# liamliaw/medical-image-segmentation-with-visual-prompts

Measured on AMD Instinct MI355X. Metric: 3D volumes/sec (96^3, bf16) training step, higher is better.
Workload: dtype bf16; 1 GPU; cfg1: swin_unetr downstream, 1-ch 96^3, batch 4/GPU, window (7, 7, 7), enc_prompt=False, dec_prompt=False, dropout 0.0, random-init weights; global_batch=4, parallelism=dp1, launch=eager (one C-ABI call per kernel)

## Files before the change

### medical-image-segmentation-with-visual-prompts_amd/csrc/common.hpp

```cpp
#pragma once
#include <hip/hip_runtime.h>
#include <stdint.h>
#include <type_traits>
#include "../../include/mivp.h"

typedef __bf16 bf16_t;
typedef __bf16 bf16x8 __attribute__((ext_vector_type(8)));
typedef __bf16 bf16x4 __attribute__((ext_vector_type(4)));
typedef float f32x4 __attribute__((ext_vector_type(4)));

#define MIVP_DEV __device__ __forceinline__

MIVP_DEV f32x4 mfma16(bf16x8 a, bf16x8 b, f32x4 c) {
    return __builtin_amdgcn_mfma_f32_16x16x32_bf16(a, b, c, 0, 0, 0);
}
MIVP_DEV bf16x8 zero8() { bf16x8 z; for (int i = 0; i < 8; ++i) z[i] = (bf16_t)0.0f; return z; }
MIVP_DEV bf16x4 zero4() { bf16x4 z; for (int i = 0; i < 4; ++i) z[i] = (bf16_t)0.0f; return z; }
MIVP_DEV f32x4 fzero4() { f32x4 z = {0.f, 0.f, 0.f, 0.f}; return z; }

MIVP_DEV bf16x8 ld8(const bf16_t* p) { return *reinterpret_cast<const bf16x8*>(p); }
MIVP_DEV bf16x4 ld4(const bf16_t* p) { return *reinterpret_cast<const bf16x4*>(p); }
MIVP_DEV void st8(bf16_t* p, bf16x8 v) { *reinterpret_cast<bf16x8*>(p) = v; }
MIVP_DEV void st4(bf16_t* p, bf16x4 v) { *reinterpret_cast<bf16x4*>(p) = v; }

// ... 19 lines not shown
    const float v = match ? s : zero;
    return excl ? -INFINITY : v;
}
MIVP_DEV float classify_logit(float s, int kcls, int rq, bool& live, float zero) {
    return classify_logit_c<-1, -2>(s, kcls, rq, live, zero);
}
constexpr float MIVP_LOG2E = 1.4426950408889634f;
constexpr float MIVP_PAD_KEY_BIAS = -30000.0f;
constexpr float MIVP_LN2 = 0.6931471805599453f;

MIVP_DEV uint32_t drop_hash(uint32_t pair_idx, uint32_t key) {
    uint32_t t = pair_idx + key;
    t ^= t >> 16;
    t = __umul24(t, 0xB5AD4Fu);
    t ^= t >> 13;
    return __umul24(t, 0x6C62B9u) + (t >> 8) + ((key << 13) | (key >> 19));
}
MIVP_DEV uint32_t drop_seed(uint32_t seed, const uint32_t* __restrict__ epoch) {
    uint32_t s = epoch ? seed + epoch[0] * 0x9E3779B1u : seed;
    s ^= s >> 16; s *= 0x85EBCA6Bu;
    s ^= s >> 13; s *= 0xC2B2AE35u;
    return s ^ (s >> 16);
}
MIVP_DEV bool drop_keep(uint32_t h, int odd, uint32_t thr) { return ((odd ? (h >> 16) : (h & 0xFFFFu)) >= thr); }
MIVP_DEV uint32_t attn_row(long bph, int q, int Nqp, int Nkp) {
    return ((uint32_t)bph * (uint32_t)Nqp + (uint32_t)q) * (uint32_t)(Nkp >> 1);
}
MIVP_DEV uint32_t attn_pair(uint32_t row, int k) { return row + (uint32_t)(k >> 1); }

typedef unsigned u32x2 __attribute__((ext_vector_type(2)));
typedef unsigned u32x4 __attribute__((ext_vector_type(4)));
MIVP_DEV int sel(bool c, int a, int b) { return c ? a : b; }
MIVP_DEV long sel(bool c, long a, long b) { return c ? a : b; }
MIVP_DEV float sel(bool c, float a, float b) { return c ? a : b; }
MIVP_DEV bf16x4 keep_if(bf16x4 v, bool ok) {
    u32x2 u = __builtin_bit_cast(u32x2, v);
    const unsigned m = 0u - (unsigned)ok;
    u[0] &= m; u[1] &= m;
    return __builtin_bit_cast(bf16x4, u);
}
MIVP_DEV bf16x8 keep_if(bf16x8 v, bool ok) {
    u32x4 u = __builtin_bit_cast(u32x4, v);
    const unsigned m = 0u - (unsigned)ok;
    u[0] &= m; u[1] &= m; u[2] &= m; u[3] &= m;
    return __builtin_bit_cast(bf16x8, u);
}
struct FastDiv {
    uint32_t m, d;
    MIVP_DEV explicit FastDiv(int div) : m(0xFFFFFFFFu / (uint32_t)div + 1u), d((uint32_t)div) {}
    MIVP_DEV int div(int n) const { return d == 1u ? n : (int)__umulhi((uint32_t)n, m); }
    MIVP_DEV int mod(int n) const { return n - div(n) * (int)d; }
};

template <int DK>
struct OperandRows {
    static constexpr int ROW = DK == 32 ? 64 : (DK + 8) * 2;
    static MIVP_DEV int off(int row, int elem) {
        if (DK == 32) return row * 64 + 16 * ((elem >> 3) ^ ((0 - (row >> 2)) & 3)) + 2 * (elem & 7);
        return row * ROW + 2 * elem;
    }
};

MIVP_DEV bf16x8 wfrag(const bf16_t* __restrict__ wf, int ks, int nt, int s, int lane) {
    return ld8(wf + ((long)(nt * ks + s) * 64 + lane) * 8);
}
template <int KSL>
struct WeightSlabs {
    static constexpr int PCS = (64 * KSL + 255) / 256;
    static constexpr int BYTES = 2 * KSL * 1024;
    bf16x8 reg[PCS];
    MIVP_DEV void fetch(const bf16_t* __restrict__ wf, int nt) {
#pragma unroll
        for (int u = 0; u < PCS; ++u) reg[u] = ld8(wf + (long)nt * KSL * 512 + 8 * min((int)threadIdx.x + 256 * u, 64 * KSL - 1));
    }
    MIVP_DEV void store(char* smem, int buf) const {
#pragma unroll
        for (int u = 0; u < PCS; ++u)
            *reinterpret_cast<bf16x8*>(smem + buf * KSL * 1024 + 16 * min((int)threadIdx.x + 256 * u, 64 * KSL - 1)) = reg[u];
    }
    static MIVP_DEV bf16x8 frag(const char* smem, int buf, int s, int lane) {
        return *reinterpret_cast<const bf16x8*>(smem + buf * KSL * 1024 + s * 1024 + 16 * lane);
    }
};

template <int KSL>
struct WeightSlabsRM {
    static constexpr int PCS = (64 * KSL + 255) / 256;
    static constexpr int BYTES = 2 * KSL * 1024;
    bf16x8 reg[PCS];
    MIVP_DEV void fetch(const bf16_t* __restrict__ w, int ld, int row0, int nrows, int ncols) {
#pragma unroll
        for (int u = 0; u < PCS; ++u) {
            const int p = threadIdx.x + 256 * u;
            const int sub = p >> 6, row = row0 + ((p & 63) >> 2), col = 32 * sub + 8 * (p & 3);
            reg[u] = (p < 64 * KSL && row < nrows && col < ncols) ? ld8(w + (long)row * ld + col) : zero8();
        }
    }
    MIVP_DEV void store(char* smem, int buf) const {
#pragma unroll
        for (int u = 0; u < PCS; ++u) {
            const int p = threadIdx.x + 256 * u;
            if (p < 64 * KSL)
                *reinterpret_cast<bf16x8*>(smem + buf * KSL * 1024 + (p >> 6) * 1024 + OperandRows<32>::off((p & 63) >> 2, 8 * (p & 3))) = reg[u];
        }
    }
    static MIVP_DEV bf16x8 frag8(const char* smem, int buf, int sub, int r, int elem) {
// ... 52 lines not shown
```

### medical-image-segmentation-with-visual-prompts_amd/csrc/swin_fwd.hip

```cpp
#include "common.hpp"
#include <cstdlib>

int mivp_tok_wide_supported(const MivpSwinDesc* d);
int mivp_tok_rows_supported(const MivpSwinDesc* d);
long mivp_tok_natural_offset(int C);
int mivp_tok_wide_qkv_fwd(const MivpSwinDesc* d, const void* x, const int32_t* tok_src, const float* ln_w, const float* ln_b,
                          const void* wqkv, void* q, void* k, void* v, hipStream_t st);
int mivp_tok_wide_proj_mlp_fwd(const MivpSwinDesc* d, const void* o, const void* x, const int32_t* tok_src, const int32_t* tok_dst,
                               const void* wproj, const float* bproj, const float* ln_w, const float* ln_b, const void* wmlp,
                               const float* bmlp, void* t1_out, void* y, hipStream_t st);

template <int KS, bool CH12>
__global__ __launch_bounds__(256, 4) void k_swin_qkv_fwd(MivpSwinDesc d, const bf16_t* __restrict__ x,
                                                      const int* __restrict__ tok_src,
                                                      const float* __restrict__ ln_w, const float* __restrict__ ln_b,
                                                      const bf16_t* __restrict__ wqkv,
                                                      bf16_t* __restrict__ q, bf16_t* __restrict__ k,
                                                      bf16_t* __restrict__ v) {
    const int lane = threadIdx.x & 63, wave = __builtin_amdgcn_readfirstlane(threadIdx.x >> 6);
    const int r = lane & 15, g = lane >> 4;
    const int C = d.C, hd = C / d.heads;
    const long T = (long)d.B * d.P * d.Nqp;
    const long tile0 = ((long)blockIdx.x * 4 + wave) * 2;

    bf16x8 xb[2][KS];
    long bp[2];
    int slot[2];
    bool live[2];
#pragma unroll
    for (int u = 0; u < 2; ++u) {
        const long t = (tile0 + u) * 16 + r;
        live[u] = t < T;
        const unsigned tt = live[u] ? (unsigned)t : 0u;
        const unsigned bpu = tt / (unsigned)d.Nqp;
        bp[u] = bpu;
        slot[u] = (int)(tt - bpu * (unsigned)d.Nqp);
        const int pw = (int)(bpu % (unsigned)d.P);
        const long b = bpu / (unsigned)d.P;
        const int src = live[u] ? tok_src[pw * d.Nqp + slot[u]] : -2;
        float xs[KS][8];
        float sum = 0.f;
#pragma unroll
        for (int s = 0; s < KS; ++s) {
            const int c = 32 * s + 8 * g;
            if (src >= 0 && c < C) {
                bf16x8 raw = ld8(x + ((b * d.vol_in + src) * (long)C + c));
#pragma unroll
                for (int i = 0; i < 8; ++i) { xs[s][i] = (float)raw[i]; sum += xs[s][i]; }
            } else {
#pragma unroll
                for (int i = 0; i < 8; ++i) xs[s][i] = 0.f;
            }
        }
        const float mean = col_sum(sum) / (float)C;
        float var = 0.f;
#pragma unroll
        for (int s = 0; s < KS; ++s) {
            if (32 * s + 8 * g < C) {
// ... 83 lines not shown
    using WR = OperandRows<32>;
    bf16x8 wreg[PCS];
    auto slab_fetch = [&](int nt) {
#pragma unroll
        for (int u = 0; u < PCS; ++u) {
            wreg[u] = ld8(wqkv + (long)nt * KS * 512 + 8 * min((int)threadIdx.x + 256 * u, 64 * KS - 1));
        }
    };
    auto slab_store = [&](int buf) {
#pragma unroll
        for (int u = 0; u < PCS; ++u) {
            *reinterpret_cast<bf16x8*>(wsm + buf * KS * 1024 + 16 * min((int)threadIdx.x + 256 * u, 64 * KS - 1)) = wreg[u];
        }
    };
    if (LDSW && nt_begin < nt_end) { slab_fetch(nt_begin); slab_store(0); __syncthreads(); }
    int o_sel = (16 * nt_begin + 4 * g) / C;
    int o_head = ((16 * nt_begin + 4 * g) - o_sel * C) / hd;
    int o_j0 = (16 * nt_begin + 4 * g) - o_sel * C - o_head * hd;
    for (int nt = nt_begin; nt < nt_end; ++nt) {
        f32x4 acc0 = fzero4(), acc1 = fzero4();
        const int nrow = 16 * nt + r;
        if (LDSW) {
            const int cur = (nt - nt_begin) & 1;
            if (nt + 1 < nt_end) slab_fetch(nt + 1);
            const char* slab = wsm + cur * KS * 1024;
#pragma unroll
            for (int s = 0; s < KS; ++s) {
                const bf16x8 a = *reinterpret_cast<const bf16x8*>(slab + s * 1024 + 16 * lane);
                acc0 = mfma16(a, xb[0][s], acc0);
                acc1 = mfma16(a, xb[1][s], acc1);
            }
            if (nt + 1 < nt_end) slab_store(cur ^ 1);
            __syncthreads();
        } else {
#pragma unroll
            for (int s = 0; s < KS; ++s) {
                const bf16x8 a = wfrag(wqkv, KS, nt, s, lane);
                acc0 = mfma16(a, xb[0][s], acc0);
                acc1 = mfma16(a, xb[1][s], acc1);
            }
        }
        const int n0 = 16 * nt + 4 * g;
        if (n0 < n_out) {
            while (o_j0 >= hd) { o_j0 -= hd; ++o_head; }
            while (o_head >= d.heads) { o_head -= d.heads; ++o_sel; }
            const int sel = o_sel, head = o_head, j0 = o_j0;
            o_j0 += 16;
            bf16_t* base = sel == 0 ? q : (sel == 1 ? k : v);
            const float sc = sel == 0 ? d.q_scale : (sel == 1 ? MIVP_LOG2E : 1.0f);
            if (live[0]) st4(base + ((bp[0] * d.heads + head) * d.Nqp + slot[0]) * (long)hd + j0, pack4(acc0 * sc));
            if (live[1]) st4(base + ((bp[1] * d.heads + head) * d.Nqp + slot[1]) * (long)hd + j0, pack4(acc1 * sc));
        }
    }
}

__global__ __launch_bounds__(256) void k_prompt_kv_fwd(MivpSwinDesc d, const float* __restrict__ prompt,
                                                       const float* __restrict__ ln_w, const float* __restrict__ ln_b,
                                                       const bf16_t* __restrict__ wqkv, bf16_t* __restrict__ kp,
                                                       bf16_t* __restrict__ vp, float* __restrict__ yln) {
    extern __shared__ __attribute__((aligned(16))) char smem[];
    float* y = reinterpret_cast<float*>(smem);
    float* red = y + d.C;
    const int t = blockIdx.x, C = d.C, hd = C / d.heads;
    const int tid = threadIdx.x;
    if (t >= d.Np) {
        for (int n = tid; n < 2 * C; n += 256) {
            const int sel = n / C, cc = n - sel * C, head = cc / hd, j = cc - head * hd;
            (sel == 0 ? kp : vp)[((long)head * d.Npp + t) * hd + j] = (bf16_t)0.0f;
        }
        return;
    }
    float part = 0.f;
    for (int c = tid; c < C; c += 256) part += prompt[(long)t * C + c];
    for (int o = 32; o > 0; o >>= 1) part += __shfl_xor(part, o);
    if ((tid & 63) == 0) red[tid >> 6] = part;
    __syncthreads();
    const float mean = (red[0] + red[1] + red[2] + red[3]) / (float)C;
    __syncthreads();
    part = 0.f;
    for (int c = tid; c < C; c += 256) { const float dv = prompt[(long)t * C + c] - mean; part += dv * dv; }
    for (int o = 32; o > 0; o >>= 1) part += __shfl_xor(part, o);
    if ((tid & 63) == 0) red[4 + (tid >> 6)] = part;
    __syncthreads();
    const float rstd = rsqrtf((red[4] + red[5] + red[6] + red[7]) / (float)C + d.ln_eps);
    for (int c = tid; c < C; c += 256) {
        const float yy = (prompt[(long)t * C + c] - mean) * rstd * ln_w[c] + ln_b[c];
        if (yln) yln[(long)t * C + c] = yy;
        y[c] = (float)(bf16_t)yy;
    }
    __syncthreads();
    for (int n = tid; n < 2 * C; n += 256) {
        const int sel = n / C, cc = n - sel * C;
        const bf16_t* wrow = wqkv + (long)((sel + 1) * C + cc) * C;
        float acc = 0.f;
        for (int c = 0; c < C; ++c) acc += y[c] * (float)wrow[c];
        const int head = cc / hd, j = cc - head * hd;
        (sel == 0 ? kp : vp)[((long)head * d.Npp + t) * hd + j] = (bf16_t)(sel == 0 ? acc * MIVP_LOG2E : acc);
    }
}

struct PromptKvJob {
    MivpSwinDesc d;
    const float* prompt; const float* ln_w; const float* ln_b; const bf16_t* wqkv; const float* ts;
    bf16_t* kp; bf16_t* vp; bf16_t* ka;
};
struct PromptKvJobs { PromptKvJob job[16]; };
// ... 658 lines not shown
            const int n0 = 16 * nt + 4 * g;
            const f32x4 w4 = *reinterpret_cast<const f32x4*>(ln_w + min(n0, C - 4));
            const f32x4 b4 = *reinterpret_cast<const f32x4*>(ln_b + min(n0, C - 4));
#pragma unroll
            for (int j = 0; j < 4; ++j) yy[j] = (bf16_t)((t1[nt][j] - mean) * rstd * w4[j] + b4[j]);
            yy = keep_if(yy, n0 < C);
        }
        y2[nt] = yy;
    }
    if (LDSW) { slab_fetch(wmlp, 0); slab_store(0); __syncthreads(); }
#pragma unroll
    for (int mt = 0; mt < CT; ++mt) {
        f32x4 acc = fzero4();
        const int nrow = 16 * mt + r;
        if (LDSW) {
            if (mt + 1 < CT) slab_fetch(wmlp, mt + 1);
            const char* slab = wsm + (mt & 1) * KS * 1024;
#pragma unroll
            for (int s = 0; s < KS; ++s) {
                acc = mfma16(*reinterpret_cast<const bf16x8*>(slab + s * 1024 + 16 * lane), cat44(y2[2 * s], y2[2 * s + 1]), acc);
            }
            if (mt + 1 < CT) slab_store((mt + 1) & 1);
            __syncthreads();
        } else {
#pragma unroll
            for (int s = 0; s < KS; ++s) {
                acc = mfma16(wfrag(wmlp, KS, mt, s, lane), cat44(y2[2 * s], y2[2 * s + 1]), acc);
            }
        }
        const int n0 = 16 * mt + 4 * g;
        const f32x4 bm4 = *reinterpret_cast<const f32x4*>(bmlp + min(n0, C - 4));
        if (n0 < C && dst >= 0) {
#pragma unroll
            for (int j = 0; j < 4; ++j) acc[j] += t1[mt][j] + bm4[j];
            st4(y + ((b * d.vol_out + dst) * (long)C + n0), pack4(acc));
        }
    }
}

static int swin_common_checks(const MivpSwinDesc* d) {
    MIVP_REQUIRE(d != nullptr);
    MIVP_REQUIRE(d->B > 0 && d->C > 0 && d->heads > 0 && d->P > 0);
    MIVP_REQUIRE(d->C % 8 == 0 && d->C % d->heads == 0 && (d->C / d->heads) % 4 == 0);
    MIVP_REQUIRE(d->Nqp % 16 == 0 && d->Nqp >= d->Nq && d->Nqp - d->Nq < 16);
    MIVP_REQUIRE((long)d->B * d->P * d->Nqp < (1L << 31));
    MIVP_REQUIRE(d->Npp % 16 == 0 && d->Npp >= d->Np);
    MIVP_REQUIRE(d->Nkp % 32 == 0 && d->Nkp >= d->Nqp + d->Npp);
    MIVP_REQUIRE(d->augp % 4 == 0 && d->augp >= d->aug);
    MIVP_REQUIRE(d->aug == d->win[0] + d->win[1] + d->win[2] - 1);
    MIVP_REQUIRE(d->Nq == d->win[0] * d->win[1] * d->win[2]);
    return MIVP_OK;
}

extern "C" int mivp_swin_qkv_fwd(const MivpSwinDesc* d, const void* x, const int32_t* tok_src, const float* ln_w,
                                 const float* ln_b, const void* wqkv, void* q, void* k, void* v,
                                 mivp_stream_t stream) {
    int rc = swin_common_checks(d);
    if (rc) return rc;
    MIVP_REQUIRE(x && tok_src && ln_w && ln_b && wqkv && q && k && v);
    if (mivp_tok_wide_supported(d)) return mivp_tok_wide_qkv_fwd(d, x, tok_src, ln_w, ln_b, wqkv, q, k, v, (hipStream_t)stream);
    const long T = (long)d->B * d->P * d->Nqp;
    const unsigned gx = (unsigned)((T + 127) / 128);
    const int KS = (d->C + 31) / 32;
    const int n_tiles = (3 * d->C + 15) / 16;
    int nsplit = (int)((4096 + 4L * gx - 1) / (4L * gx));
    if (nsplit > n_tiles / 3) nsplit = n_tiles / 3;
    if (nsplit < 1) nsplit = 1;
    const dim3 grid(gx, (unsigned)nsplit);
    hipStream_t st = (hipStream_t)stream;
#define LAUNCH_QKV2(K, CH) hipLaunchKernelGGL((k_swin_qkv_fwd<K, CH>), grid, dim3(256), 0, st, *d, (const bf16_t*)x, tok_src, \
                                              ln_w, ln_b, (const bf16_t*)wqkv, (bf16_t*)q, (bf16_t*)k, (bf16_t*)v)
#define LAUNCH_QKV(K) LAUNCH_QKV2(K, false)
    const bool ch12 = d->C == 48 && d->heads == 4 && nsplit == 1 && d->Nqp % 32 == 0;
    switch (KS) {
        case 1: LAUNCH_QKV(1); break;
        case 2: if (ch12) LAUNCH_QKV2(2, true); else LAUNCH_QKV(2); break;
        case 3: LAUNCH_QKV(3); break;
        case 4: LAUNCH_QKV(4); break;
        case 6: LAUNCH_QKV(6); break;
        default: mivp_set_error("swin_qkv_fwd: C/32 not in {1,2,3,4,6}"); return MIVP_EUNSUPPORTED;
    }
#undef LAUNCH_QKV
    return mivp_check_launch("swin_qkv_fwd");
}

extern "C" int mivp_prompt_kv_fwd(const MivpSwinDesc* d, const float* prompt, const float* ln_w, const float* ln_b,
                                  const void* wqkv, void* kp, void* vp, float* yln, mivp_stream_t stream) {
    int rc = swin_common_checks(d);
    if (rc) return rc;
    MIVP_REQUIRE(d->Np > 0 && prompt && ln_w && ln_b && wqkv && kp && vp);
    hipLaunchKernelGGL(k_prompt_kv_fwd, dim3(d->Npp), dim3(256), (d->C + 8) * sizeof(float), (hipStream_t)stream, *d,
                       prompt, ln_w, ln_b, (const bf16_t*)wqkv, (bf16_t*)kp, (bf16_t*)vp, yln);
    return mivp_check_launch("prompt_kv_fwd");
}

extern "C" int mivp_prompt_kv_fwd_multi(int32_t n, const MivpSwinDesc* d, const float* const* prompt, const float* const* ln_w,
                                        const float* const* ln_b, const void* const* wqkv, const float* const* ts,
                                        void* const* kp, void* const* vp, void* const* ka, mivp_stream_t stream) {
    MIVP_REQUIRE(n > 0 && n <= 16 && d && prompt && ln_w && ln_b && wqkv && ts && kp && vp && ka);
    PromptKvJobs jobs;
    int rows = 0;
    size_t lds = 0;
    for (int i = 0; i < n; ++i) {
        int rc = swin_common_checks(&d[i]);
        if (rc) return rc;
        MIVP_REQUIRE(d[i].Np > 0 && prompt[i] && ln_w[i] && ln_b[i] && wqkv[i] && ts[i] && kp[i] && vp[i] && ka[i]);
        jobs.job[i] = PromptKvJob{d[i], prompt[i], ln_w[i], ln_b[i], (const bf16_t*)wqkv[i], ts[i], (bf16_t*)kp[i], (bf16_t*)vp[i],
                                  (bf16_t*)ka[i]};
        rows = d[i].Npp > rows ? d[i].Npp : rows;
        const size_t need = (d[i].C + 8) * sizeof(float);
        lds = need > lds ? need : lds;
    }
    hipLaunchKernelGGL(k_prompt_kv_fwd_multi, dim3(rows, n), dim3(256), lds, (hipStream_t)stream, jobs);
    return mivp_check_launch("prompt_kv_fwd_multi");
}

extern "C" int mivp_relbias_aug(const MivpSwinDesc* d, const float* t_h, const float* t_w, const float* t_d,
                                const float* ts, void* qa, void* ka, mivp_stream_t stream) {
    int rc = swin_common_checks(d);
    if (rc) return rc;
    MIVP_REQUIRE(t_h && t_w && t_d && qa && ka);
    MIVP_REQUIRE(d->Np == 0 || ts != nullptr);
    hipLaunchKernelGGL(k_relbias_aug, dim3(d->heads + 1, 8), dim3(256), 0, (hipStream_t)stream, *d, t_h, t_w, t_d, ts,
                       (bf16_t*)qa, (bf16_t*)ka);
    return mivp_check_launch("relbias_aug");
}
// ... 107 lines not shown
```

### medical-image-segmentation-with-visual-prompts_amd/csrc/swin_tok_wide.hip

```cpp
#include "common.hpp"
#include <cstdlib>

namespace {

template <int CT>
struct WideGeom {
    static constexpr int C = 16 * CT;
    static constexpr int KP = (C + 31) / 32 * 32;
    static constexpr int KS = KP / 32;
    static constexpr int NCG = (CT % 4 == 0) ? 4 : (CT % 2 == 0 ? 2 : 1);
    static constexpr int NTG = 4 / NCG;
    static constexpr int NCT = CT / NCG;
    static constexpr int ROWS = 32 * NTG;
    static constexpr int TPR = 256 / ROWS;
    static constexpr int XPT = C / 8 / TPR;
    static_assert(CT % NCG == 0 && (C / 8) % TPR == 0, "even splits");
};

template <int K>
struct RowImg {
    static constexpr int ROWB = 2 * K + 16;
    static MIVP_DEV bf16x8 frag(const char* img, int row, int k0) { return *reinterpret_cast<const bf16x8*>(img + row * ROWB + 2 * k0); }
    static MIVP_DEV bf16x4 get4(const char* img, int row, int k0) { return *reinterpret_cast<const bf16x4*>(img + row * ROWB + 2 * k0); }
    static MIVP_DEV void put4(char* img, int row, int k0, bf16x4 v) { *reinterpret_cast<bf16x4*>(img + row * ROWB + 2 * k0) = v; }
    static MIVP_DEV void put8(char* img, int row, int k0, bf16x8 v) { *reinterpret_cast<bf16x8*>(img + row * ROWB + 2 * k0) = v; }
};

struct RowTok { long tt, bp, b; int slot, pw; bool live; };
MIVP_DEV RowTok row_token(const MivpSwinDesc& d, long t) {
    RowTok ti;
    const long T = (long)d.B * d.P * d.Nqp;
    ti.live = t < T;
    const unsigned tu = ti.live ? (unsigned)t : 0u;
    const unsigned bpu = tu / (unsigned)d.Nqp;
    ti.tt = tu;
    ti.bp = bpu;
    ti.slot = (int)(tu - bpu * (unsigned)d.Nqp);
    ti.pw = (int)(bpu % (unsigned)d.P);
    ti.b = bpu / (unsigned)d.P;
    return ti;
}
template <int TPR>
MIVP_DEV float row_sum(float v) {
#pragma unroll
    for (int o = 1; o < TPR; o <<= 1) v += __shfl_xor(v, o);
    return v;
}
MIVP_DEV void to_f32(bf16x8 v, float (&out)[8]) {
#pragma unroll
    for (int e = 0; e < 8; ++e) out[e] = (float)v[e];
}

template <int CT>
struct FlatRows {
    using G = WideGeom<CT>;
    static constexpr int PPR = G::C / 8, N = G::XPT;
    static_assert(G::ROWS * PPR == 256 * N, "pieces split evenly over the threads");
    int prow[N], col[N];
    RowTok tk[N];
    MIVP_DEV FlatRows(const MivpSwinDesc& d, long row0, int tid) {
#pragma unroll
        for (int i = 0; i < N; ++i) {
            const int P = tid + 256 * i;
            prow[i] = P / PPR;
            col[i] = 8 * (P - prow[i] * PPR);
            tk[i] = row_token(d, row0 + prow[i]);
        }
    }
};
template <int CT> constexpr bool flat_rows() { return CT == 3; }

template <int C, int NTG>
struct HeadMajor {
    long gbase[NTG];
    bool glive[NTG];
    int hd, hd4, heads;
    long head_stride;
    FastDiv by_chunk, by_hd4, by_heads;
    static constexpr int PER_GRAN = 24 * C;
    static constexpr int PPT = PER_GRAN * NTG / 256;
    MIVP_DEV HeadMajor(const MivpSwinDesc& d, long row0)
        : hd(C / d.heads), hd4(C / d.heads / 4), heads(d.heads), head_stride((long)d.Nqp * (C / d.heads)),
          by_chunk(8 * (C / d.heads)), by_hd4(C / d.heads / 4), by_heads(d.heads) {
        const long T = (long)d.B * d.P * d.Nqp;
#pragma unroll
        for (int gi = 0; gi < NTG; ++gi) {
            const long t0 = row0 + 32 * gi;
            glive[gi] = t0 < T;
            const unsigned tu = glive[gi] ? (unsigned)t0 : 0u;
            const unsigned bp = tu / (unsigned)d.Nqp, slot0 = tu - bp * (unsigned)d.Nqp;
            gbase[gi] = ((long)bp * heads * d.Nqp + slot0) * hd;
        }
    }
    template <class F>
    MIVP_DEV void each(int tid, F&& visit) const {
#pragma unroll
        for (int i = 0; i < PPT; ++i) {
            const int P = tid + 256 * i;
            const int gran = P / PER_GRAN, pg = P - gran * PER_GRAN;
// ... 348 lines not shown
            for (int e = 0; e < 8; ++e) sum += ts[i][e];
        }
        const float mean = row_sum<TPR>(sum) / (float)C;
        float var = 0.f;
#pragma unroll
        for (int i = 0; i < XPT; ++i)
#pragma unroll
            for (int e = 0; e < 8; ++e) { const float dvv = ts[i][e] - mean; var += dvv * dvv; }
        const float rstd = rsqrtf(row_sum<TPR>(var) / (float)C + d.ln_eps);
#pragma unroll
        for (int i = 0; i < XPT; ++i) {
            const int c = 8 * (sub + TPR * i);
            const f32x4 w0 = *reinterpret_cast<const f32x4*>(ln_w + c), w1 = *reinterpret_cast<const f32x4*>(ln_w + c + 4);
            const f32x4 b0 = *reinterpret_cast<const f32x4*>(ln_b + c), b1 = *reinterpret_cast<const f32x4*>(ln_b + c + 4);
            bf16x8 yy;
#pragma unroll
            for (int e = 0; e < 4; ++e) {
                yy[e] = (bf16_t)((ts[i][e] - mean) * rstd * w0[e] + b0[e]);
                yy[4 + e] = (bf16_t)((ts[i][4 + e] - mean) * rstd * w1[e] + b1[e]);
            }
            RI::put8(Aimg, row, c, yy);
        }
    }
    __syncthreads();
    {
#pragma unroll
        for (int j = 0; j < NCT; ++j) {
            const int nt = cg + NCG * j, n0 = 16 * nt + 4 * g;
            const f32x4 bm4 = *reinterpret_cast<const f32x4*>(bmlp + n0);
            f32x4 a0 = fzero4(), a1 = fzero4();
#pragma unroll
            for (int s = 0; s < KS; ++s) {
                bf16x8 a;
                if constexpr (PREW) a = wa[j][s]; else a = wfrag(wmlp, KS, nt, s, lane);
                a0 = mfma16(a, RI::frag(Aimg, R0, 32 * s + 8 * g), a0);
                a1 = mfma16(a, RI::frag(Aimg, R1, 32 * s + 8 * g), a1);
            }
            RI::put4(Ximg, R0, n0, pack4(a0 + t1[j][0] + bm4));
            RI::put4(Ximg, R1, n0, pack4(a1 + t1[j][1] + bm4));
        }
    }
    __syncthreads();
    if (FLAT) {
#pragma unroll
        for (int i = 0; i < XPT; ++i) {
            const int P = tid + 256 * i, prow = P / (C / 8), col = 8 * (P - prow * (C / 8));
            if (fdst[i] >= 0) st8(y + ((long)fb[i] * d.vol_out + fdst[i]) * (long)C + col, RI::frag(Ximg, prow, col));
        }
    } else if (dst >= 0) {
        const long yoff = (ti.b * d.vol_out + dst) * (long)C;
#pragma unroll
        for (int i = 0; i < XPT; ++i) st8(y + yoff + 8 * (sub + TPR * i), RI::frag(Ximg, row, 8 * (sub + TPR * i)));
    }
}

template <int CT>
__global__ __launch_bounds__(256, 3) void k_proj_mlp_bwd_wide(MivpSwinDesc d, const bf16_t* __restrict__ dy, const int* __restrict__ tok_dst,
                                                              const bf16_t* __restrict__ t1, const float* __restrict__ ln_w,
                                                              const bf16_t* __restrict__ wmlp_t, const bf16_t* __restrict__ wproj_t,
                                                              bf16_t* __restrict__ d_o, bf16_t* __restrict__ d_t1) {
    using G = WideGeom<CT>;
    constexpr int C = G::C, KS = G::KS, ROWS = G::ROWS, TPR = G::TPR, NCG = G::NCG, NCT = G::NCT, XPT = G::XPT;
    using RI = RowImg<G::KP>;
    extern __shared__ __attribute__((aligned(16))) char smem[];
    char* Dimg = smem;
    char* Timg = Dimg + ROWS * RI::ROWB;
    float* stat = reinterpret_cast<float*>(Timg + ROWS * RI::ROWB);
    float* red = stat + 2 * ROWS;
    const int tid = threadIdx.x, lane = tid & 63, wave = __builtin_amdgcn_readfirstlane(tid >> 6);
    const int r = lane & 15, g = lane >> 4;
    const long row0 = (long)blockIdx.x * ROWS;
    const int row = tid / TPR, sub = tid % TPR;
    const RowTok ti = row_token(d, row0 + row);
    const uint32_t proj_key = drop_seed(d.proj_seed, d.seed_epoch);
    const bool drop = d.proj_drop_thr != 0;
    {
        const int dst = sel(ti.live, tok_dst[ti.pw * d.Nqp + ti.slot], -1);
        const long yoff = (ti.b * d.vol_out + max(dst, 0)) * (long)C;
        bf16x8 dr[XPT], tr[XPT];
#pragma unroll
        for (int i = 0; i < XPT; ++i) {
            dr[i] = ld8(dy + yoff + 8 * (sub + TPR * i));
            tr[i] = ld8(t1 + ti.tt * (long)C + 8 * (sub + TPR * i));
        }
        float ts[XPT][8], sum = 0.f;
#pragma unroll
        for (int i = 0; i < XPT; ++i) {
            const bf16x8 tv = keep_if(tr[i], ti.live);
            RI::put8(Dimg, row, 8 * (sub + TPR * i), keep_if(dr[i], dst >= 0));
            RI::put8(Timg, row, 8 * (sub + TPR * i), tv);
            to_f32(tv, ts[i]);
#pragma unroll
            for (int e = 0; e < 8; ++e) sum += ts[i][e];
        }
        const float mean = row_sum<TPR>(sum) / (float)C;
        float var = 0.f;
#pragma unroll
        for (int i = 0; i < XPT; ++i)
#pragma unroll
            for (int e = 0; e < 8; ++e) { const float dvv = ts[i][e] - mean; var += dvv * dvv; }
        const float rstd = rsqrtf(row_sum<TPR>(var) / (float)C + d.ln_eps);
        if (sub == 0) {
            stat[2 * row] = mean;
            stat[2 * row + 1] = rstd;
            for (int c = C; c < G::KP; c += 8) { RI::put8(Dimg, row, c, zero8()); RI::put8(Timg, row, c, zero8()); }
        }
// ... 326 lines not shown
    PackJobs jobs;
    jobs.n = 0;
    jobs.C = C;
    jobs.w[0] = wq; jobs.w[1] = wk; jobs.w[2] = wv; jobs.w[3] = wproj; jobs.w[4] = wmlp;
    const int ct = (C + 15) / 16, ks = (C + 31) / 32, ks3 = (3 * 16 * ct + 31) / 32, ct3 = (3 * C + 15) / 16;
    auto add = [&](void* out, int src, int transposed, int kind, int rows, int cols, int k_steps) {
        if (!out) return;
        PackJob& j = jobs.job[jobs.n++];
        j.out = (bf16_t*)out; j.src = src; j.transposed = transposed; j.kind = kind; j.rows = rows; j.cols = cols; j.k_steps = k_steps;
        j.elems = kind == 0 ? (long)rows * cols : (long)((rows + 15) / 16) * k_steps * 512;
    };
    const long img = (long)ct * ks * 512;
    add(wqkv_rm, 0, 0, 0, 3 * C, C, 0);
    add(wqkv_f, 0, 0, 1, 3 * C, C, ks);
    add(wproj_f, 1, 0, 1, C, C, ks);
    add(wmlp_f, 2, 0, 2, C, C, ks);
    if (with_natural && wmlp_f) add((bf16_t*)wmlp_f + img, 2, 0, 1, C, C, ks);
    add(wqkv_t, 0, 1, 1, C, 3 * C, ks3);
    add(wmlp_t, 2, 1, 1, C, C, ks);
    add(wproj_t, 1, 1, 2, C, C, ks);
    if (with_natural && wproj_t) add((bf16_t*)wproj_t + img, 1, 1, 1, C, C, ks);
    (void)ct3;
    long total = 0;
    for (int j = 0; j < jobs.n; ++j) total += jobs.job[j].elems;
    if (total == 0) return MIVP_OK;
    const unsigned grid = (unsigned)((total + 255) / 256 < 4096 ? (total + 255) / 256 : 4096);
    hipLaunchKernelGGL(k_pack_block_weights, dim3(grid), dim3(256), 0, (hipStream_t)stream, jobs);
    return mivp_check_launch("pack_block_weights");
}

extern "C" int mivp_pack_weight_frags(const void* w, int32_t rows, int32_t cols, int32_t k_steps, int32_t paired, void* out,
                                      mivp_stream_t stream) {
    MIVP_REQUIRE(w && out && rows > 0 && cols > 0 && k_steps >= (cols + 31) / 32);
    const long total = (long)((rows + 15) / 16) * k_steps * 512;
    const unsigned grid = (unsigned)((total + 255) / 256 < 2048 ? (total + 255) / 256 : 2048);
    hipLaunchKernelGGL(k_pack_weight_frags, dim3(grid), dim3(256), 0, (hipStream_t)stream, (const bf16_t*)w, rows, cols, k_steps,
                       paired, (bf16_t*)out, total);
    return mivp_check_launch("pack_weight_frags");
}

int mivp_tok_wide_supported(const MivpSwinDesc* d) {
    const int hd = d->C / d->heads;
    if (!(d->C == 48 || d->C == 96 || d->C == 192 || d->C == 384)) return 0;
    static const bool off = getenv("MIVP_NO_WIDE_TOKEN_KERNELS") != nullptr;
    if (off) return 0;
    if (d->C == 48 && !getenv("MIVP_C48_QKV_ROW_KERNELS")) return 0;
    return (hd % 4 == 0 && d->Nqp % 32 == 0 && 8 * hd < 65536 && 72 * d->C < 65536) ? 1 : 0;
}
int mivp_tok_rows_supported(const MivpSwinDesc* d) {
    if (mivp_tok_wide_supported(d)) return 1;
    static const bool off = getenv("MIVP_NO_WIDE_TOKEN_KERNELS") != nullptr;
    return (!off && d->C == 48) ? 1 : 0;
}
long mivp_tok_natural_offset(int C) { return (long)(C / 16) * ((C + 31) / 32) * 512; }

#define ROWS_SWITCH(LAUNCH)                                                                  \
    switch (d->C) {                                                                          \
        case 48: LAUNCH(3); break;                                                           \
        case 96: LAUNCH(6); break;                                                           \
        case 192: LAUNCH(12); break;                                                         \
        case 384: LAUNCH(24); break;                                                         \
        default: mivp_set_error("tok_rows: C not in {48, 96, 192, 384}"); return MIVP_EUNSUPPORTED; \
    }
#define WIDE_SWITCH(LAUNCH)                                                                  \
    switch (d->C) {                                                                          \
        case 96: LAUNCH(6); break;                                                           \
        case 192: LAUNCH(12); break;                                                         \
        case 384: LAUNCH(24); break;                                                         \
        default: mivp_set_error("tok_wide: C not in {96, 192, 384}"); return MIVP_EUNSUPPORTED; \
    }
#define WIDE_GRID(CTV) dim3((unsigned)((T + WideGeom<CTV>::ROWS - 1) / WideGeom<CTV>::ROWS))

int mivp_tok_wide_qkv_fwd(const MivpSwinDesc* d, const void* x, const int32_t* tok_src, const float* ln_w, const float* ln_b,
                          const void* wqkv, void* q, void* k, void* v, hipStream_t st) {
    const long T = (long)d->B * d->P * d->Nqp;
#define L_W(CTV)                                                                                                             \
    do {                                                                                                                     \
        const size_t lds = lds_qkv_fwd<CTV>();                                                                               \
        MIVP_LDS_OPT_IN(k_qkv_fwd_wide<CTV>, lds);                                                                           \
        hipLaunchKernelGGL((k_qkv_fwd_wide<CTV>), WIDE_GRID(CTV), dim3(256), lds, st, *d, (const bf16_t*)x, tok_src, ln_w,   \
                           ln_b, (const bf16_t*)wqkv, (bf16_t*)q, (bf16_t*)k, (bf16_t*)v);                                   \
    } while (0)
    static const bool no_ws = getenv("MIVP_QKV_FWD_STREAMED_WEIGHTS") != nullptr;
    const int hd = d->C / d->heads;
    if (!no_ws && (d->C == 96 || d->C == 192) && hd % 4 == 0 && d->Nqp % 16 == 0 && d->Nqp >= 64) {
#define L_WS(CTV)                                                                                                            \
    do {                                                                                                                     \
        const size_t lds = (size_t)64 * RowImg<WideGeom<CTV>::KP>::ROWB;                                                     \
        hipLaunchKernelGGL((k_qkv_fwd_ws<CTV>), dim3((unsigned)((T + 63) / 64)), dim3(256), lds, st, *d, (const bf16_t*)x,   \
                           tok_src, ln_w, ln_b, (const bf16_t*)wqkv, (bf16_t*)q, (bf16_t*)k, (bf16_t*)v);                    \
    } while (0)
        if (d->C == 96) L_WS(6); else L_WS(12);
#undef L_WS
        return mivp_check_launch("swin_qkv_fwd(weight-stationary)");
    }
    ROWS_SWITCH(L_W)
#undef L_W
    return mivp_check_launch("swin_qkv_fwd(wide)");
}

int mivp_tok_wide_proj_mlp_fwd(const MivpSwinDesc* d, const void* o, const void* x, const int32_t* tok_src, const int32_t* tok_dst,
                               const void* wproj, const float* bproj, const float* ln_w, const float* ln_b, const void* wmlp,
                               const float* bmlp, void* t1_out, void* y, hipStream_t st) {
    const long T = (long)d->B * d->P * d->Nqp;
#define L_W(CTV)                                                                                                              \
    do {                                                                                                                      \
        const size_t lds = lds_proj_mlp_fwd<CTV>();                                                                           \
        MIVP_LDS_OPT_IN(k_proj_mlp_fwd_wide<CTV>, lds);                                                                       \
        hipLaunchKernelGGL((k_proj_mlp_fwd_wide<CTV>), WIDE_GRID(CTV), dim3(256), lds, st, *d, (const bf16_t*)o,              \
                           (const bf16_t*)x, tok_src, tok_dst, (const bf16_t*)wproj, bproj, ln_w, ln_b, (const bf16_t*)wmlp,  \
                           bmlp, (bf16_t*)t1_out, (bf16_t*)y);                                                                \
    } while (0)
    ROWS_SWITCH(L_W)
#undef L_W
    return mivp_check_launch("swin_proj_mlp_fwd(wide)");
}

int mivp_tok_wide_proj_mlp_bwd(const MivpSwinDesc* d, const void* dy, const int32_t* tok_dst, const void* t1, const float* ln_w,
                               const void* wmlp_t, const void* wproj_t, void* d_o, void* d_t1, hipStream_t st) {
    const long T = (long)d->B * d->P * d->Nqp;
#define L_W(CTV)                                                                                                             \
    do {                                                                                                                     \
        const size_t lds = lds_proj_mlp_bwd<CTV>();                                                                          \
        MIVP_LDS_OPT_IN(k_proj_mlp_bwd_wide<CTV>, lds);                                                                      \
        hipLaunchKernelGGL((k_proj_mlp_bwd_wide<CTV>), WIDE_GRID(CTV), dim3(256), lds, st, *d, (const bf16_t*)dy, tok_dst,   \
                           (const bf16_t*)t1, ln_w, (const bf16_t*)wmlp_t, (const bf16_t*)wproj_t, (bf16_t*)d_o,             \
                           (bf16_t*)d_t1);                                                                                   \
    } while (0)
    ROWS_SWITCH(L_W)
#undef L_W
    return mivp_check_launch("swin_proj_mlp_bwd(wide)");
}

int mivp_tok_wide_qkv_bwd(const MivpSwinDesc* d, const void* dq, const void* dk, const void* dv, const void* x, const int32_t* tok_src,
                          const float* ln_w, const void* wqkv_t, const void* d_t1, void* dx, void* dn_out, hipStream_t st) {
    const long T = (long)d->B * d->P * d->Nqp;
#define L_W(CTV)                                                                                                             \
    do {                                                                                                                     \
        const size_t lds = lds_qkv_bwd<CTV>();                                                                               \
        MIVP_LDS_OPT_IN(k_qkv_bwd_wide<CTV>, lds);                                                                           \
        hipLaunchKernelGGL((k_qkv_bwd_wide<CTV>), WIDE_GRID(CTV), dim3(256), lds, st, *d, (const bf16_t*)dq, (const bf16_t*)dk, \
                           (const bf16_t*)dv, (const bf16_t*)x, tok_src, ln_w, (const bf16_t*)wqkv_t, (const bf16_t*)d_t1,   \
                           (bf16_t*)dx, (bf16_t*)dn_out);                                                                    \
    } while (0)
    ROWS_SWITCH(L_W)
#undef L_W
    return mivp_check_launch("swin_qkv_bwd(wide)");
}
```

Measured before the change: 1709 volumes/s.

## Add persistent C=48 kernels for swin qkv and proj-MLP forward

Adds persistent-grid variants of the C=48 QKV and proj+MLP forward kernels, sized to the resident block count per compute unit. Each block stages the weights in LDS once and then walks a contiguous range of work items, software-pipelining the loads of the next item's indices and rows behind the current item's compute. The QKV variant also reorders its output stores through ds_bpermute so each lane writes contiguous pieces. This trades per-block weight reloads and launch tail effects for more complex code, higher LDS use and possible occupancy limits. It is enabled by default and can be turned off with an environment variable.

New measurement: 1726 volumes/s (median of 6 runs). 1.0% higher.

```diff
diff --git a/medical-image-segmentation-with-visual-prompts_amd/csrc/common.hpp b/medical-image-segmentation-with-visual-prompts_amd/csrc/common.hpp
--- a/medical-image-segmentation-with-visual-prompts_amd/csrc/common.hpp
+++ b/medical-image-segmentation-with-visual-prompts_amd/csrc/common.hpp
@@ -95,6 +95,13 @@
     MIVP_DEV int mod(int n) const { return n - div(n) * (int)d; }
 };
 
+MIVP_DEV void persistent_items(int n_items, int& first, int& end) {
+    unsigned vb = blockIdx.x;
+    if ((gridDim.x & 7u) == 0u) vb = (blockIdx.x & 7u) * (gridDim.x >> 3) + (blockIdx.x >> 3);
+    first = (int)((long)vb * n_items / gridDim.x);
+    end = (int)((long)(vb + 1) * n_items / gridDim.x);
+}
+
 template <int DK>
 struct OperandRows {
     static constexpr int ROW = DK == 32 ? 64 : (DK + 8) * 2;
diff --git a/medical-image-segmentation-with-visual-prompts_amd/csrc/swin_fwd.hip b/medical-image-segmentation-with-visual-prompts_amd/csrc/swin_fwd.hip
--- a/medical-image-segmentation-with-visual-prompts_amd/csrc/swin_fwd.hip
+++ b/medical-image-segmentation-with-visual-prompts_amd/csrc/swin_fwd.hip
@@ -4,6 +4,8 @@
 int mivp_tok_wide_supported(const MivpSwinDesc* d);
 int mivp_tok_rows_supported(const MivpSwinDesc* d);
 long mivp_tok_natural_offset(int C);
+int mivp_tok_persistent_enabled();
+int mivp_tok_resident_grid(int per_cu, long n_items);
 int mivp_tok_wide_qkv_fwd(const MivpSwinDesc* d, const void* x, const int32_t* tok_src, const float* ln_w, const float* ln_b,
                           const void* wqkv, void* q, void* k, void* v, hipStream_t st);
 int mivp_tok_wide_proj_mlp_fwd(const MivpSwinDesc* d, const void* o, const void* x, const int32_t* tok_src, const int32_t* tok_dst,
@@ -193,6 +195,167 @@
             if (live[1]) st4(base + ((bp[1] * d.heads + head) * d.Nqp + slot[1]) * (long)hd + j0, pack4(acc1 * sc));
         }
     }
+}
+
+__global__ __launch_bounds__(256, 4) void k_swin_qkv_fwd_c48_persistent(MivpSwinDesc d, const bf16_t* __restrict__ x,
+                                                                        const int* __restrict__ tok_src,
+                                                                        const float* __restrict__ ln_w, const float* __restrict__ ln_b,
+                                                                        const bf16_t* __restrict__ wqkv,
+                                                                        bf16_t* __restrict__ q, bf16_t* __restrict__ k,
+                                                                        bf16_t* __restrict__ v, int n_items) {
+    constexpr int KS = 2, NF = 9 * KS;
+    __shared__ __attribute__((aligned(16))) char wsm[NF * 1024];
+    __shared__ __attribute__((aligned(16))) float lnsm[2][64];
+    const int tid = threadIdx.x, lane = tid & 63, wave = __builtin_amdgcn_readfirstlane(tid >> 6);
+    const int r = lane & 15, g = lane >> 4;
+    const int C = d.C;
+    const unsigned Nqp = (unsigned)d.Nqp;
+    const int n_units = (int)(((long)d.B * d.P * d.Nqp) >> 5);
+    int first, end;
+    persistent_items(n_items, first, end);
+    for (int i = tid; i < NF * 64; i += 256) *reinterpret_cast<bf16x8*>(wsm + 16 * i) = ld8(wqkv + 8 * i);
+    if (tid < 128) {
+        const int c = tid & 63;
+        lnsm[tid >> 6][c] = c < C ? (tid < 64 ? ln_w : ln_b)[c] : 0.f;
+    }
+    __syncthreads();
+
+    auto load_idx = [&](int item, int (&src)[2], unsigned& b) {
+        const unsigned tt = 32u * (unsigned)min(item * 4 + wave, n_units - 1);
+        const unsigned bpu = (unsigned)__builtin_amdgcn_readfirstlane((int)(tt / Nqp));
+        const unsigned slot0 = tt - bpu * Nqp, pw = bpu % (unsigned)d.P;
+        b = bpu / (unsigned)d.P;
+#pragma unroll
+        for (int u = 0; u < 2; ++u) src[u] = tok_src[pw * Nqp + slot0 + 16 * u + r];
+    };
+    auto load_rows = [&](const int (&src)[2], unsigned b, bf16x8 (&raw)[2][KS]) {
+#pragma unroll
+        for (int u = 0; u < 2; ++u)
+#pragma unroll
+            for (int s = 0; s < KS; ++s) {
+                const int c = 32 * s + 8 * g;
+                raw[u][s] = ld8(x + (((long)b * d.vol_in + max(src[u], 0)) * (long)C + (c < C ? c : 0)));
+            }
+    };
+
+    const int dl = lane < 48 ? lane : lane - 16, rq = dl / 3, gq = dl - 3 * rq;
+    int src_addr[4];
+    bool from_b[4];
+#pragma unroll
+    for (int h = 0; h < 4; ++h) {
+        const int ch = 12 * h + 4 * gq;
+        src_addr[h] = 4 * (rq + 16 * ((ch & 15) >> 2));
+        from_b[h] = (ch >> 4) != ((12 * h) >> 4);
+    }
+
+    int src_a[2], src_b[2];
+    unsigned b_a, b_b;
+    bf16x8 raw_b[2][KS];
+    load_idx(first, src_b, b_b);
+    load_rows(src_b, b_b, raw_b);
+    load_idx(first + 1, src_a, b_a);
+    auto turn = [&](int item) -> bool {
+        bf16x8 raw[2][KS];
+        int src2[2];
+#pragma unroll
+        for (int u = 0; u < 2; ++u) {
+            src2[u] = src_b[u];
+#pragma unroll
+            for (int s = 0; s < KS; ++s) raw[u][s] = raw_b[u][s];
+        }
+        load_rows(src_a, b_a, raw_b);
+        src_b[0] = src_a[0]; src_b[1] = src_a[1]; b_b = b_a;
+        load_idx(item + 2, src_a, b_a);
+        const int unit = item * 4 + wave;
+        if (unit >= n_units) return false;
+
+        bf16x8 xb[2][KS];
+#pragma unroll
+        for (int u = 0; u < 2; ++u) {
+            const int src = src2[u];
+            float xs[KS][8];
+            float sum = 0.f;
+#pragma unroll
+            for (int s = 0; s < KS; ++s) {
+                const int c = 32 * s + 8 * g;
+                if (src >= 0 && c < C) {
+#pragma unroll
+                    for (int i = 0; i < 8; ++i) { xs[s][i] = (float)raw[u][s][i]; sum += xs[s][i]; }
+                } else {
+#pragma unroll
+                    for (int i = 0; i < 8; ++i) xs[s][i] = 0.f;
+                }
+            }
+            const float mean = col_sum(sum) / (float)C;
+            float var = 0.f;
+#pragma unroll
+            for (int s = 0; s < KS; ++s) {
+                if (32 * s + 8 * g < C) {
+#pragma unroll
+                    for (int i = 0; i < 8; ++i) { const float dv = xs[s][i] - mean; var += dv * dv; }
+                }
+            }
+            const float rstd = rsqrtf(col_sum(var) / (float)C + d.ln_eps);
+#pragma unroll
+            for (int s = 0; s < KS; ++s) {
+                const int c = 32 * s + 8 * g;
+                bf16x8 y = zero8();
+                if (src >= -1 && c < C) {
+#pragma unroll
+                    for (int i = 0; i < 8; ++i) y[i] = (bf16_t)((xs[s][i] - mean) * rstd * lnsm[0][c + i] + lnsm[1][c + i]);
+                }
+                xb[u][s] = y;
+            }
+        }
+
+        long chunk[2];
+        {
+            const unsigned tt = 32u * (unsigned)unit;
+            const unsigned bpu = (unsigned)__builtin_amdgcn_readfirstlane((int)(tt / Nqp));
+#pragma unroll
+            for (int u = 0; u < 2; ++u) chunk[u] = ((long)bpu * 4 * Nqp + (tt + 16 * u - bpu * Nqp)) * 12;
+        }
+#pragma unroll
+        for (int sl = 0; sl < 3; ++sl) {
+            const float sc = sl == 0 ? d.q_scale : (sl == 1 ? MIVP_LOG2E : 1.0f);
+            u32x2 pk[3][2];
+#pragma unroll
+            for (int t = 0; t < 3; ++t) {
+                f32x4 acc0 = fzero4(), acc1 = fzero4();
+#pragma unroll
+                for (int s = 0; s < KS; ++s) {
+                    const bf16x8 a = *reinterpret_cast<const bf16x8*>(wsm + ((3 * sl + t) * KS + s) * 1024 + 16 * lane);
+                    acc0 = mfma16(a, xb[0][s], acc0);
+                    acc1 = mfma16(a, xb[1][s], acc1);
+                }
+                pk[t][0] = __builtin_bit_cast(u32x2, pack4(acc0 * sc));
+                pk[t][1] = __builtin_bit_cast(u32x2, pack4(acc1 * sc));
+            }
+            bf16_t* base = sl == 0 ? q : (sl == 1 ? k : v);
+#pragma unroll
+            for (int h = 0; h < 4; ++h) {
+                const int ta = (12 * h) >> 4, tb = (12 * h + 8) >> 4;
+#pragma unroll
+                for (int u = 0; u < 2; ++u) {
+                    u32x2 piece;
+                    piece[0] = (unsigned)__builtin_amdgcn_ds_bpermute(src_addr[h], (int)pk[ta][u][0]);
+                    piece[1] = (unsigned)__builtin_amdgcn_ds_bpermute(src_addr[h], (int)pk[ta][u][1]);
+                    if (tb != ta) {
+                        const unsigned b0 = (unsigned)__builtin_amdgcn_ds_bpermute(src_addr[h], (int)pk[tb][u][0]);
+                        const unsigned b1 = (unsigned)__builtin_amdgcn_ds_bpermute(src_addr[h], (int)pk[tb][u][1]);
+                        piece[0] = from_b[h] ? b0 : piece[0];
+                        piece[1] = from_b[h] ? b1 : piece[1];
+                    }
+                    char* cb = reinterpret_cast<char*>(base + (chunk[u] + (long)h * Nqp * 12));
+                    *reinterpret_cast<u32x2*>(cb + (unsigned)(8 * dl)) = piece;
+                }
+            }
+        }
+        return true;
+    };
+    if (first < end && turn(first))
+        for (int item = first + 1; item < end; ++item)
+            if (!turn(item)) break;
 }
 
 __global__ __launch_bounds__(256) void k_prompt_kv_fwd(MivpSwinDesc d, const float* __restrict__ prompt,
@@ -957,6 +1120,19 @@
     return MIVP_OK;
 }
 
+static int qkv_persistent_per_cu() {
+    static int per_cu = 0;
+    if (per_cu == 0) {
+        int n = 0;
+        if (hipOccupancyMaxActiveBlocksPerMultiprocessor(&n, k_swin_qkv_fwd_c48_persistent, 256, 0) != hipSuccess || n < 1) n = 4;
+        per_cu = n > 6 ? 6 : n;
+    }
+    return per_cu;
+}
+extern "C" int mivp_tok_persistent_grid(int32_t kernel, int64_t n_items) {
+    return mivp_tok_resident_grid(kernel == 0 ? qkv_persistent_per_cu() : 3, (long)n_items);
+}
+
 extern "C" int mivp_swin_qkv_fwd(const MivpSwinDesc* d, const void* x, const int32_t* tok_src, const float* ln_w,
                                  const float* ln_b, const void* wqkv, void* q, void* k, void* v,
                                  mivp_stream_t stream) {
@@ -977,6 +1153,13 @@
                                               ln_w, ln_b, (const bf16_t*)wqkv, (bf16_t*)q, (bf16_t*)k, (bf16_t*)v)
 #define LAUNCH_QKV(K) LAUNCH_QKV2(K, false)
     const bool ch12 = d->C == 48 && d->heads == 4 && nsplit == 1 && d->Nqp % 32 == 0;
+    if (ch12 && mivp_tok_persistent_enabled()) {
+        const int pgrid = mivp_tok_resident_grid(qkv_persistent_per_cu(), (long)gx);
+        if (pgrid <= 0) return MIVP_ELAUNCH;
+        hipLaunchKernelGGL(k_swin_qkv_fwd_c48_persistent, dim3((unsigned)pgrid), dim3(256), 0, st, *d, (const bf16_t*)x, tok_src,
+                           ln_w, ln_b, (const bf16_t*)wqkv, (bf16_t*)q, (bf16_t*)k, (bf16_t*)v, (int)gx);
+        return mivp_check_launch("swin_qkv_fwd(persistent)");
+    }
     switch (KS) {
         case 1: LAUNCH_QKV(1); break;
         case 2: if (ch12) LAUNCH_QKV2(2, true); else LAUNCH_QKV(2); break;
diff --git a/medical-image-segmentation-with-visual-prompts_amd/csrc/swin_tok_wide.hip b/medical-image-segmentation-with-visual-prompts_amd/csrc/swin_tok_wide.hip
--- a/medical-image-segmentation-with-visual-prompts_amd/csrc/swin_tok_wide.hip
+++ b/medical-image-segmentation-with-visual-prompts_amd/csrc/swin_tok_wide.hip
@@ -45,6 +45,11 @@
 #pragma unroll
     for (int o = 1; o < TPR; o <<= 1) v += __shfl_xor(v, o);
     return v;
+}
+MIVP_DEV float mul_then_add(float a, float b, float c) {
+#pragma clang fp contract(off)
+    const float p = a * b;
+    return p + c;
 }
 MIVP_DEV void to_f32(bf16x8 v, float (&out)[8]) {
 #pragma unroll
@@ -499,6 +504,196 @@
 #pragma unroll
         for (int i = 0; i < XPT; ++i) st8(y + yoff + 8 * (sub + TPR * i), RI::frag(Ximg, row, 8 * (sub + TPR * i)));
     }
+}
+
+template <int CT>
+__global__ __launch_bounds__(256, 3) void k_proj_mlp_fwd_persistent(MivpSwinDesc d, const bf16_t* __restrict__ o, const bf16_t* __restrict__ x,
+                                                                    const int* __restrict__ tok_src, const int* __restrict__ tok_dst,
+                                                                    const bf16_t* __restrict__ wproj, const float* __restrict__ bproj,
+                                                                    const float* __restrict__ ln_w, const float* __restrict__ ln_b,
+                                                                    const bf16_t* __restrict__ wmlp, const float* __restrict__ bmlp,
+                                                                    bf16_t* __restrict__ t1_out, bf16_t* __restrict__ y, int n_items) {
+    using G = WideGeom<CT>;
+    static_assert(flat_rows<CT>() && G::NCG == 1, "piece-major rows, one column group (C = 48)");
+    constexpr int C = G::C, KS = G::KS, ROWS = G::ROWS, TPR = G::TPR, NCT = G::NCT, XPT = G::XPT, PPR = C / 8;
+    using RI = RowImg<G::KP>;
+    extern __shared__ __attribute__((aligned(16))) char smem[];
+    char* Aimg = smem;
+    char* Ximg = Aimg + ROWS * RI::ROWB;
+    const int tid = threadIdx.x, lane = tid & 63, wave = __builtin_amdgcn_readfirstlane(tid >> 6);
+    const int r = lane & 15, g = lane >> 4;
+    const int row = tid / TPR, sub = tid % TPR;
+    const long T = (long)d.B * d.P * d.Nqp;
+    const unsigned PN = (unsigned)d.P * (unsigned)d.Nqp;
+    const uint32_t proj_key = drop_seed(d.proj_seed, d.seed_epoch);
+    int first, end;
+    persistent_items(n_items, first, end);
+    if (first >= end) return;
+
+    constexpr int WIMG = NCT * KS * 1024;
+    char* Wp = Ximg + ROWS * RI::ROWB;
+    char* Wm = Wp + WIMG;
+    for (int i = tid; i < WIMG / 16; i += 256) {
+        *reinterpret_cast<bf16x8*>(Wp + 16 * i) = ld8(wproj + 8 * i);
+        *reinterpret_cast<bf16x8*>(Wm + 16 * i) = ld8(wmlp + 8 * i);
+    }
+    float* Vb = reinterpret_cast<float*>(Wm + WIMG);
+    const float *bproj_s = Vb, *bmlp_s = Vb + C, *ln_w_s = Vb + 2 * C, *ln_b_s = Vb + 3 * C;
+    if (tid < C) { Vb[tid] = bproj[tid]; Vb[C + tid] = bmlp[tid]; Vb[2 * C + tid] = ln_w[tid]; Vb[3 * C + tid] = ln_b[tid]; }
+    int prow[XPT], col[XPT];
+#pragma unroll
+    for (int i = 0; i < XPT; ++i) {
+        const int P = tid + 256 * i;
+        prow[i] = P / PPR;
+        col[i] = 8 * (P - prow[i] * PPR);
+    }
+    if (G::KP != C && sub == 0)
+        for (int c = C; c < G::KP; c += 8) RI::put8(Aimg, row, c, zero8());
+
+    auto load_idx = [&](int item, int (&xsrc)[XPT], int (&ydst)[XPT]) {
+        const long row0 = (long)min(item, n_items - 1) * ROWS;
+#pragma unroll
+        for (int i = 0; i < XPT; ++i) {
+            const long t = row0 + prow[i];
+            const bool live = t < T;
+            const unsigned tu = live ? (unsigned)t : 0u;
+            const unsigned bb = tu / PN, in_b = tu - bb * PN;
+            const int src = sel(live, tok_src[in_b], -2), dst = sel(live, tok_dst[in_b], -1);
+            xsrc[i] = sel(src >= 0, (int)bb * d.vol_in + src, src);
+            ydst[i] = sel(dst >= 0, (int)bb * d.vol_out + dst, dst);
+        }
+    };
+    auto load_rows = [&](int item, const int (&xsrc)[XPT], bf16x8 (&orow)[XPT], bf16x8 (&xr)[XPT]) {
+        const long row0 = (long)min(item, n_items - 1) * ROWS;
+#pragma unroll
+        for (int i = 0; i < XPT; ++i) {
+            const long t = row0 + prow[i];
+            const long tu = t < T ? t : 0;
+            orow[i] = ld8(o + tu * C + col[i]);
+            xr[i] = ld8(x + (long)max(xsrc[i], 0) * (long)C + col[i]);
+        }
+    };
+
+    int xsrc_b[XPT], ydst_b[XPT];
+    bf16x8 o_b[XPT], x_b[XPT];
+    load_idx(first, xsrc_b, ydst_b);
+    load_rows(first, xsrc_b, o_b, x_b);
+    const int R0 = wave * 32 + r, R1 = R0 + 16;
+    auto turn = [&](int item, bool first_turn) {
+        const long row0 = (long)item * ROWS;
+        int ydst[XPT];
+        if (!first_turn) __syncthreads();
+#pragma unroll
+        for (int i = 0; i < XPT; ++i) {
+            RI::put8(Aimg, prow[i], col[i], keep_if(o_b[i], row0 + prow[i] < T));
+            RI::put8(Ximg, prow[i], col[i], keep_if(x_b[i], xsrc_b[i] >= 0));
+            ydst[i] = ydst_b[i];
+        }
+        load_idx(item + 1, xsrc_b, ydst_b);
+        __syncthreads();
+        bf16x4 t1[NCT][2];
+        {
+#pragma unroll
+            for (int j = 0; j < NCT; ++j) {
+                const int n0 = 16 * j + 4 * g;
+                const f32x4 bp4 = *reinterpret_cast<const f32x4*>(bproj_s + n0);
+                f32x4 a0 = fzero4(), a1 = fzero4();
+#pragma unroll
+                for (int s = 0; s < KS; ++s) {
+                    const bf16x8 a = *reinterpret_cast<const bf16x8*>(Wp + (j * KS + s) * 1024 + 16 * lane);
+                    a0 = mfma16(a, RI::frag(Aimg, R0, 32 * s + 8 * g), a0);
+                    a1 = mfma16(a, RI::frag(Aimg, R1, 32 * s + 8 * g), a1);
+                }
+                const bf16x4 s0 = RI::get4(Ximg, R0, n0), s1 = RI::get4(Ximg, R1, n0);
+                if (d.proj_drop_thr) {
+                    const uint32_t p0 = (uint32_t)(((row0 + R0) * C + n0) >> 1), p1 = (uint32_t)(((row0 + R1) * C + n0) >> 1);
+                    const uint32_t h00 = drop_hash(p0, proj_key), h01 = drop_hash(p0 + 1, proj_key);
+                    const uint32_t h10 = drop_hash(p1, proj_key), h11 = drop_hash(p1 + 1, proj_key);
+                    const float sc = d.proj_drop_scale;
+                    const float k0[4] = {drop_keep(h00, 0, d.proj_drop_thr) ? sc : 0.f, drop_keep(h00, 1, d.proj_drop_thr) ? sc : 0.f,
+                                         drop_keep(h01, 0, d.proj_drop_thr) ? sc : 0.f, drop_keep(h01, 1, d.proj_drop_thr) ? sc : 0.f};
+                    const float k1[4] = {drop_keep(h10, 0, d.proj_drop_thr) ? sc : 0.f, drop_keep(h10, 1, d.proj_drop_thr) ? sc : 0.f,
+                                         drop_keep(h11, 0, d.proj_drop_thr) ? sc : 0.f, drop_keep(h11, 1, d.proj_drop_thr) ? sc : 0.f};
+#pragma unroll
+                    for (int e = 0; e < 4; ++e) {
+                        a0[e] = (float)(bf16_t)__builtin_fmaf(a0[e] + bp4[e], k0[e], (float)s0[e]);
+                        a1[e] = (float)(bf16_t)((j == NCT - 1 && e == 3) ? mul_then_add(a1[e] + bp4[e], k1[e], (float)s1[e])
+                                                                         : __builtin_fmaf(a1[e] + bp4[e], k1[e], (float)s1[e]));
+                    }
+                } else {
+#pragma unroll
+                    for (int e = 0; e < 4; ++e) {
+                        a0[e] = (float)(bf16_t)(a0[e] + bp4[e] + (float)s0[e]);
+                        a1[e] = (float)(bf16_t)(a1[e] + bp4[e] + (float)s1[e]);
+                    }
+                }
+                t1[j][0] = pack4(a0);
+                t1[j][1] = pack4(a1);
+                RI::put4(Ximg, R0, n0, t1[j][0]);
+                RI::put4(Ximg, R1, n0, t1[j][1]);
+            }
+        }
+        __syncthreads();
+        {
+            const bool live = row0 + row < T;
+            float ts[XPT][8], sum = 0.f;
+#pragma unroll
+            for (int i = 0; i < XPT; ++i) {
+                const bf16x8 raw = RI::frag(Ximg, row, 8 * (sub + TPR * i));
+                if (t1_out && live) st8(t1_out + (row0 + row) * (long)C + 8 * (sub + TPR * i), raw);
+                to_f32(raw, ts[i]);
+#pragma unroll
+                for (int e = 0; e < 8; ++e) sum += ts[i][e];
+            }
+            const float mean = row_sum<TPR>(sum) / (float)C;
+            float var = 0.f;
+#pragma unroll
+            for (int i = 0; i < XPT; ++i)
+#pragma unroll
+                for (int e = 0; e < 8; ++e) { const float dvv = ts[i][e] - mean; var += dvv * dvv; }
+            const float rstd = rsqrtf(row_sum<TPR>(var) / (float)C + d.ln_eps);
+#pragma unroll
+            for (int i = 0; i < XPT; ++i) {
+                const int c = 8 * (sub + TPR * i);
+                const f32x4 w0 = *reinterpret_cast<const f32x4*>(ln_w_s + c), w1 = *reinterpret_cast<const f32x4*>(ln_w_s + c + 4);
+                const f32x4 b0 = *reinterpret_cast<const f32x4*>(ln_b_s + c), b1 = *reinterpret_cast<const f32x4*>(ln_b_s + c + 4);
+                bf16x8 yy;
+#pragma unroll
+                for (int e = 0; e < 4; ++e) {
+                    yy[e] = (bf16_t)((ts[i][e] - mean) * rstd * w0[e] + b0[e]);
+                    yy[4 + e] = (bf16_t)((ts[i][4 + e] - mean) * rstd * w1[e] + b1[e]);
+                }
+                RI::put8(Aimg, row, c, yy);
+            }
+        }
+        __syncthreads();
+        load_rows(item + 1, xsrc_b, o_b, x_b);
+        {
+#pragma unroll
+            for (int j = 0; j < NCT; ++j) {
+                const int n0 = 16 * j + 4 * g;
+                const f32x4 bm4 = *reinterpret_cast<const f32x4*>(bmlp_s + n0);
+                f32x4 a0 = fzero4(), a1 = fzero4();
+#pragma unroll
+                for (int s = 0; s < KS; ++s) {
+                    const bf16x8 a = *reinterpret_cast<const bf16x8*>(Wm + (j * KS + s) * 1024 + 16 * lane);
+                    a0 = mfma16(a, RI::frag(Aimg, R0, 32 * s + 8 * g), a0);
+                    a1 = mfma16(a, RI::frag(Aimg, R1, 32 * s + 8 * g), a1);
+                }
+                f32x4 u0, u1;
+#pragma unroll
+                for (int e = 0; e < 4; ++e) { u0[e] = (float)t1[j][0][e]; u1[e] = (float)t1[j][1][e]; }
+                RI::put4(Ximg, R0, n0, pack4(a0 + u0 + bm4));
+                RI::put4(Ximg, R1, n0, pack4(a1 + u1 + bm4));
+            }
+        }
+        __syncthreads();
+#pragma unroll
+        for (int i = 0; i < XPT; ++i)
+            if (ydst[i] >= 0) st8(y + (long)ydst[i] * (long)C + col[i], RI::frag(Ximg, prow[i], col[i]));
+    };
+    turn(first, true);
+    for (int item = first + 1; item < end; ++item) turn(item, false);
 }
 
 template <int CT>
@@ -931,6 +1126,22 @@
     static const bool off = getenv("MIVP_NO_WIDE_TOKEN_KERNELS") != nullptr;
     return (!off && d->C == 48) ? 1 : 0;
 }
+int mivp_tok_persistent_enabled() { return getenv("MIVP_TOK_NO_PERSISTENT") == nullptr ? 1 : 0; }
+int mivp_tok_resident_grid(int per_cu, long n_items) {
+    static int cus[64];
+    int dev = 0;
+    if (hipGetDevice(&dev) != hipSuccess || dev < 0 || dev >= 64) { mivp_set_error("tok_persistent: no current device"); return -1; }
+    if (cus[dev] == 0) {
+        int n = 0;
+        if (hipDeviceGetAttribute(&n, hipDeviceAttributeMultiprocessorCount, dev) != hipSuccess || n <= 0) {
+            mivp_set_error("tok_persistent: the device reports no compute units");
+            return -1;
+        }
+        cus[dev] = n;
+    }
+    const long cap = (long)cus[dev] * per_cu;
+    return (int)(n_items < cap ? n_items : cap);
+}
 long mivp_tok_natural_offset(int C) { return (long)(C / 16) * ((C + 31) / 32) * 512; }
 
 #define ROWS_SWITCH(LAUNCH)                                                                  \
@@ -990,6 +1201,15 @@
                            (const bf16_t*)x, tok_src, tok_dst, (const bf16_t*)wproj, bproj, ln_w, ln_b, (const bf16_t*)wmlp,  \
                            bmlp, (bf16_t*)t1_out, (bf16_t*)y);                                                                \
     } while (0)
+    if (d->C == 48 && mivp_tok_persistent_enabled()) {
+        const long n_items = (T + WideGeom<3>::ROWS - 1) / WideGeom<3>::ROWS;
+        const int pgrid = mivp_tok_resident_grid(3, n_items);
+        if (pgrid <= 0) return MIVP_ELAUNCH;
+        hipLaunchKernelGGL((k_proj_mlp_fwd_persistent<3>), dim3((unsigned)pgrid), dim3(256), lds_proj_mlp_fwd<3>() + 2 * 6 * 1024 + 4 * 48 * sizeof(float), st, *d,
+                           (const bf16_t*)o, (const bf16_t*)x, tok_src, tok_dst, (const bf16_t*)wproj, bproj, ln_w, ln_b,
+                           (const bf16_t*)wmlp, bmlp, (bf16_t*)t1_out, (bf16_t*)y, (int)n_items);
+        return mivp_check_launch("swin_proj_mlp_fwd(persistent)");
+    }
     ROWS_SWITCH(L_W)
 #undef L_W
     return mivp_check_launch("swin_proj_mlp_fwd(wide)");
```
